# cczls1991/DL_Biomass

Hardware: NVIDIA B200
Metric: train tree-clouds/sec @10k pts (higher is better)
Workload: dtype bf16

## Files before the change

### dl_biomass_b200/csrc/sa_tc.cu

```cuda
#include <cuda.h>
#include <math.h>

#include "tc_common.cuh"

namespace b2pn {
namespace tc {

constexpr int R = 128;
constexpr int KC = 64;
constexpr int NUM_EPI = 256;
constexpr int NUM_LOAD = 128;
constexpr int LOAD_GROUPS = 2;
constexpr int MMA_WARP = (NUM_EPI + LOAD_GROUPS * NUM_LOAD) / 32;
constexpr int NT = NUM_EPI + LOAD_GROUPS * NUM_LOAD + 32;
constexpr int NT_TMA = 2 * NUM_EPI + 64;
constexpr int PROD_WARP_TMA = MMA_WARP + 1;
constexpr int NT_WIDE = 2 * NUM_EPI + 32 + NUM_LOAD;
constexpr int B_BYTES = R * LINE_BYTES;

constexpr unsigned GI_NONE = 0x00ffffffu;
__device__ __forceinline__ int gi_seg(unsigned b) { return (int)(b & 0xffffffu); }
__device__ __forceinline__ bool gi_none(unsigned b) { return (b & 0xffffffu) == 0xffffffu; }
__device__ __forceinline__ int gi_slot0(unsigned b) { return (int)((b >> 24) & 7u) << 3; }
__device__ __forceinline__ int gi_nv(unsigned b) { return (int)((b >> 27) & 15u); }
// ... 244 lines not shown
    }
    static __device__ __forceinline__ uint64_t b_desc(uint32_t b_saddr, int ks) { return smem_desc_sw128(b_saddr + ks * 32, 16, ATOM_BYTES); }
};

constexpr int GATHER_ROWS = 64;
__global__ void __launch_bounds__(256) gather_l1_tc_kernel(GatherLoaderTC gl, const int64_t *rows_dev, int kg, int64_t ld,
                                                          __nv_bfloat16 *G)
{
    extern __shared__ __align__(16) unsigned char gth_smem[];
    __nv_bfloat16 *S = reinterpret_cast<__nv_bfloat16 *>(gth_smem);
    const int64_t rows = rows_dev ? *rows_dev : gl.rm.rows;
    gl.resolve(rows);
    const int64_t r0 = (int64_t)blockIdx.x * GATHER_ROWS;
    if (r0 >= (rows + 127) / 128 * 128) return;
    const int kg8 = (kg + 7) & ~7;
    const int rl = threadIdx.x & 63, q = threadIdx.x >> 6;
    gl.set_row(r0 + rl);
    for (int kk = q * 8; kk < kg8; kk += 32) {
        const uint4 v = gl.chunk(kk);
        const __nv_bfloat16 *e = reinterpret_cast<const __nv_bfloat16 *>(&v);
#pragma unroll
        for (int j = 0; j < 8; ++j) S[(kk + j) * GATHER_ROWS + rl] = e[j];
    }
    __syncthreads();
    for (int i = threadIdx.x; i < kg8 * 8; i += 256) {
        const int k = i >> 3, part = i & 7;
        if (k < kg)
            *reinterpret_cast<uint4 *>(G + (int64_t)k * ld + r0 + part * 8) =
                *reinterpret_cast<const uint4 *>(S + k * GATHER_ROWS + part * 8);
    }
}

template <int MODE>
struct FeatSource {
    static constexpr bool USES_TMA = false;
    static constexpr bool SCATTER = false;
    RowMapTC rm;
    const __nv_bfloat16 *t;
    int C;
    int64_t ld;
    int act;
    int ones_line;
    const float *gamma;
    const float *beta;
    int out_fmt;
    __device__ __forceinline__ uint4 pack_out(const float (&f)[8]) const { return out_fmt == FMT_F16 ? pack8h(f) : pack8(f); }
    __device__ __forceinline__ void resolve(int64_t r) { rm.resolve(r); }
    __device__ __forceinline__ uint4 chunk_i(int ch, int64_t r8, unsigned inf) const
    {
        const int nv = gi_nv(inf);
        float f[8];
        if (ch == ones_line) {
#pragma unroll
            for (int e = 0; e < 8; ++e) f[e] = e < nv ? 1.f : 0.f;
            return pack_out(f);
        }
        const bool live = ch < C && nv > 0;
        uint4 raw = make_uint4(0u, 0u, 0u, 0u);
        if (!live) return raw;
        raw = __ldg(reinterpret_cast<const uint4 *>(t + (int64_t)ch * ld + r8));
        if (MODE == 0 && nv == 8 && out_fmt == FMT_F16) return raw;
        unpack8h(raw, f);
        float ga = 1.f, be = 0.f;
        if (MODE != 0) {
            ga = gamma[ch];
            be = beta[ch];
        }
#pragma unroll
        for (int e = 0; e < 8; ++e) {
            float v = f[e];
            if (MODE != 0) {
                v = fmaf(v, ga, be);
                if (act == B2PN_ACT_RELU) v = fmaxf(v, 0.f);
            }
            f[e] = e < nv ? v : 0.f;
        }
        return pack_out(f);
    }
};

struct TmaSource {
    static constexpr bool USES_TMA = true;
    static constexpr bool SCATTER = false;
    RowMapTC rm;
    __device__ __forceinline__ void resolve(int64_t r) { rm.resolve(r); }
    __device__ __forceinline__ uint4 chunk_i(int, int64_t, unsigned) const { return make_uint4(0u, 0u, 0u, 0u); }
};

struct RouteSource {
    static constexpr bool USES_TMA = false;
    RowMapTC rm;
    const float *dout;
    const int32_t *arg;
    int C;
    __device__ __forceinline__ void resolve(int64_t r) { rm.resolve(r); }
    static constexpr bool SCATTER = true;
    int vec;
    struct Quad {
        int4 a;
        float4 d;
    };
    __device__ __forceinline__ bool starts(unsigned inf, int ch4) const { return ch4 < C && gi_nv(inf) > 0 && gi_slot0(inf) == 0; }
    __device__ __forceinline__ void load_quad(unsigned inf, int ch4, Quad &q) const
    {
        const bool first = starts(inf, ch4);
        const int64_t idx = first ? (int64_t)gi_seg(inf) * C + ch4 : 0;
        if (vec) {
            q.a = __ldg(reinterpret_cast<const int4 *>(arg + idx));
            q.d = __ldg(reinterpret_cast<const float4 *>(dout + idx));
        } else {
            const int64_t last = (first ? (int64_t)gi_seg(inf) * C : 0) + C - 1;
            q.a = make_int4(__ldg(arg + idx), __ldg(arg + min(idx + 1, last)), __ldg(arg + min(idx + 2, last)), __ldg(arg + min(idx + 3, last)));
            q.d = make_float4(__ldg(dout + idx), __ldg(dout + min(idx + 1, last)), __ldg(dout + min(idx + 2, last)),
                              __ldg(dout + min(idx + 3, last)));
        }
    }
    __device__ __forceinline__ void store_quad(const Quad &q, bool first, int ch4, int g, uint32_t blk, int l0) const
    {
        const int a[4] = {q.a.x, q.a.y, q.a.z, q.a.w};
        const float d[4] = {q.d.x, q.d.y, q.d.z, q.d.w};
#pragma unroll
        for (int e = 0; e < 4; ++e) {
            const unsigned row = (unsigned)(g * 8 + a[e]);
            const unsigned ok = (first && ch4 + e < C && a[e] >= 0 && row < 64u) ? 1u : 0u;
            const uint32_t line = (uint32_t)(l0 + e);
            const uint32_t addr = blk + line * LINE_BYTES + ((((row >> 3) & 7u) ^ (line & 7u)) << 4) + ((row & 7u) << 1);
            const unsigned short gb = __bfloat16_as_ushort(__float2bfloat16(d[e]));
            asm volatile("{\n\t.reg .pred p;\n\tsetp.ne.u32 p, %2, 0;\n\t@p st.shared.b16 [%0], %1;\n\t}" ::"r"(addr), "h"(gb), "r"(ok)
                         : "memory");
        }
    }
    template <int NTHR = NUM_LOAD>
    static __device__ __forceinline__ void zero_tile(uint32_t base, int bytes, int lt)
    {
        for (int o = lt * 16; o < bytes; o += NTHR * 16)
            asm volatile("st.shared.v4.b32 [%0], {%1, %1, %1, %1};" ::"r"(base + (uint32_t)o), "r"(0u) : "memory");
    }
    template <int NTHR = NUM_LOAD>
    static __device__ __forceinline__ void group_barrier(int id) { asm volatile("bar.sync %0, %1;" ::"r"(id), "n"(NTHR) : "memory"); }
    __device__ __forceinline__ uint4 chunk_i(int ch, int64_t, unsigned inf) const
    {
        const bool live = ch < C && gi_nv(inf) > 0;
        const int64_t idx = live ? (int64_t)gi_seg(inf) * C + ch : 0;
        const int a = __ldg(arg + idx) - gi_slot0(inf);
        const float d = __ldg(dout + idx);
        const bool hit = live && a >= 0 && a < 8;
        const unsigned short gb = __bfloat16_as_ushort(__float2bfloat16(d));
        const unsigned w = (a & 1) ? ((unsigned)gb << 16) : (unsigned)gb;
        const int q = hit ? (a >> 1) : -1;
        uint4 v;
        v.x = q == 0 ? w : 0u;
        v.y = q == 1 ? w : 0u;
        v.z = q == 2 ? w : 0u;
        v.w = q == 3 ? w : 0u;
        return v;
    }
};

template <class SRC, bool WIDE_ = false>
struct FeatLoaderTC {
    static constexpr bool B_MN = true;
    static constexpr bool USES_TMA = false;
    static constexpr bool WIDE = WIDE_;
    static constexpr bool PIPELINED = SRC::SCATTER;
    SRC src;
    int64_t row0;
    unsigned inf[8];
    static constexpr int PIPE_GROUPS = 2;
    unsigned qinf[2], qraw1[2], qraw2[2], qdead1, qdead2;
    struct Item {
        typename SRC::Quad q[2];
        unsigned first;
    };
// ... 802 lines not shown
    static constexpr bool USES_TMA = true;
    int c;
    int ones_box;
    const float *fix_gamma;
    const float *fix_beta;
    int fix_act;
    __device__ __forceinline__ uint4 convert(const uint4 &raw, int c16, int ng) const
    {
        const int ch = ng * 256 + (c16 >> 3);
        if (fix_gamma == nullptr || ch >= c) return f16_to_bf16_chunk(raw);
        const float ga = __ldg(fix_gamma + ch), be = __ldg(fix_beta + ch);
        float f[8];
        unpack8h(raw, f);
#pragma unroll
        for (int e = 0; e < 8; ++e) {
            f[e] = fmaf(f[e], ga, be);
            if (fix_act == B2PN_ACT_RELU) f[e] = fmaxf(f[e], 0.f);
        }
        return pack8(f);
    }
    static __host__ __device__ int bytes(int nb_lines) { return ((nb_lines + 63) / 64) * 64 * LINE_BYTES; }
    __device__ __forceinline__ void resolve(int64_t) {}
    __device__ __forceinline__ void fill(uint8_t *, int, int64_t, int, int, const unsigned (&)[8]) {}
    __device__ __forceinline__ int landed_lines(int ng) const
    {
        const int ch0 = ng * 256;
        const int left = c - ch0;
        const int boxes = left <= 0 ? 0 : ((left < 256 ? left : 256) + 63) >> 6;
        const bool ones_here = ones_box && c >= ch0 && c < ch0 + 256;
        const int tensor_lines = boxes * 64;
        return ones_here ? max(tensor_lines, c - ch0 + 16) : tensor_lines;
    }
    __device__ __forceinline__ unsigned fill_tma(uint8_t *B, int64_t r0, int ng, const TmaMap *map_x, const TmaMap *map_v,
                                                 uint64_t *bar) const
    {
        const int ch0 = ng * 256;
        const int left = c - ch0;
        const int boxes = left <= 0 ? 0 : ((left < 256 ? left : 256) + 63) >> 6;
        const bool ones_here = ones_box && c >= ch0 && c < ch0 + 256;
        const unsigned bytes = (unsigned)((boxes * 64 + (ones_here ? 16 : 0)) * LINE_BYTES);
        mbar_expect_tx(bar, bytes);
        for (int blk = 0; blk < boxes; ++blk) tma_load_2d(B + blk * (64 * LINE_BYTES), map_x, (int)r0, ch0 + blk * 64, bar);
        if (ones_here) tma_load_2d(B + (c - ch0) * LINE_BYTES, map_v, (int)r0, 0, bar);
        return bytes;
    }
    static __device__ __forceinline__ uint64_t b_desc(uint32_t b_saddr, int ks) { return smem_desc_sw128(b_saddr + ks * 32, 16, ATOM_BYTES); }
};

struct LineFillGather {
    static constexpr bool B_MN = true;
    static constexpr bool USES_TMA = false;
    GatherLoaderTC g;
    static __host__ __device__ int bytes(int nb_lines) { return ((nb_lines + 63) / 64) * 64 * LINE_BYTES; }
    __device__ __forceinline__ void resolve(int64_t r) { g.resolve(r); }
    __device__ __forceinline__ void fill(uint8_t *B, int lt, int64_t r0, int ng, int nb_lines, const unsigned (&inf)[8])
    {
        const int rl = lt >> 1, half = lt & 1;
        g.set_row(r0 + rl);
        const int nblk = (nb_lines + 63) / 64;
        for (int blk = 0; blk < nblk; ++blk) {
#pragma unroll
            for (int c = 0; c < 4; ++c) {
                const int cc = half * 4 + c;
                *reinterpret_cast<uint4 *>(B + blk * (64 * LINE_BYTES) + line_chunk_off(rl, cc)) =
                    g.chunk(ng * 256 + blk * 64 + cc * 8);
            }
        }
    }
    static __device__ __forceinline__ uint64_t b_desc(uint32_t b_saddr, int ks)
    {
        return smem_desc_sw128(b_saddr + ks * (16 * LINE_BYTES), 64 * LINE_BYTES, ATOM_BYTES);
    }
};

template <int MTA>
struct DwPlan {
    static constexpr int A_BYTES = MTA * 128 * LINE_BYTES;
    static constexpr int MAX_STAGES = 8;
    static constexpr int SMEM_BUDGET = 222 * 1024;
};

template <int MTA, class YS, class XF>
__global__ void __launch_bounds__(NT, 1) tc_dw_kernel(const DwParams p, YS ys, XF xf, const __grid_constant__ TmaMap tmap_y,
                                                       const __grid_constant__ TmaMap tmap_x, const __grid_constant__ TmaMap tmap_v)
{
    using P = DwPlan<MTA>;
    const int nst = p.stages, sbytes = p.stage_bytes;
    extern __shared__ uint8_t smem_raw[];
    uint8_t *smem = reinterpret_cast<uint8_t *>((reinterpret_cast<uintptr_t>(smem_raw) + 1023) & ~(uintptr_t)1023);
    uint64_t *full = reinterpret_cast<uint64_t *>(smem + nst * sbytes);
    uint64_t *empty = full + nst;
    uint64_t *done = empty + nst;
    uint64_t *xland = done + 1;
    uint32_t *tmem_holder = reinterpret_cast<uint32_t *>(xland + nst);

    const int tid = threadIdx.x, warp = tid >> 5, lane = tid & 31;
    const int split = blockIdx.x, mg = blockIdx.y, ng = blockIdx.z;
    constexpr int TCOLS = MTA * 256;
    const int64_t rows = p.rows_dev ? *p.rows_dev : p.rows;
    ys.resolve(rows);
    xf.resolve(rows);
    const int64_t chunks = (rows + 63) / 64;
    const int64_t cps = (chunks + gridDim.x - 1) / gridDim.x;
    const int64_t c_beg = (int64_t)split * cps;
    const int64_t c_end = min(chunks, c_beg + cps);
    const int64_t nchunks = c_end > c_beg ? c_end - c_beg : 0;
    const int nb_lines = min(256, p.nbl_total - ng * 256);

    if (tid == 0) {
        for (int s = 0; s < nst; ++s) {
            mbar_init(&full[s], YS::SCATTER ? 2 * NUM_LOAD : NUM_LOAD);
            mbar_init(&empty[s], 1);
            mbar_init(&xland[s], 1);
        }
        mbar_init(done, 1);
        fence_barrier_init();
    }
    if (warp == MMA_WARP) tmem_alloc<TCOLS>(tmem_holder);
    tc_fence_before();
    __syncthreads();
    tc_fence_after();
    const uint32_t tmem_base = *tmem_holder;

    constexpr bool ANY_TMA = YS::USES_TMA || XF::USES_TMA;
    constexpr bool DEDICATED = ANY_TMA && !YS::SCATTER;
    auto issue = [&](int64_t i) {
        const int s = (int)(i % nst);
        const uint32_t ph = (uint32_t)(i / nst) & 1u;
        uint8_t *A = smem + s * sbytes;
        uint8_t *B = A + P::A_BYTES;
        const int64_t r0 = (c_beg + i) * 64;
        mbar_wait(&empty[s], ph ^ 1u);
        if constexpr (YS::USES_TMA) {
            mbar_expect_tx(&full[s], P::A_BYTES);
#pragma unroll
            for (int m = 0; m < MTA * 2; ++m)
                tma_load_2d(A + m * (64 * LINE_BYTES), &tmap_y, (int)r0, mg * (MTA * 128) + m * 64, &full[s]);
        }
        if constexpr (XF::USES_TMA) {
            xf.fill_tma(B, r0, ng, &tmap_x, &tmap_v, &xland[s]);
            mbar_arrive(&xland[s]);
        }
    };
    constexpr int NG = DEDICATED ? LOAD_GROUPS + 1 : LOAD_GROUPS;
    if ((warp >= NUM_EPI / 32 && warp < MMA_WARP) || (DEDICATED && warp < 4)) {
        const int grp = warp < 4 ? LOAD_GROUPS : (tid - NUM_EPI) / NUM_LOAD;
        const int lt = warp < 4 ? tid : (tid - NUM_EPI) % NUM_LOAD;
        auto load_inf = [&](unsigned (&inf)[8], int64_t r0) {
            if (ys.rm.seg_mode) {
#pragma unroll
                for (int g = 0; g < 8; ++g) inf[g] = ys.rm.info(r0 + g * 8);
            } else {
#pragma unroll
                for (int g = 0; g < 8; ++g) inf[g] = ys.rm.info_slots(r0 + g * 8);
            }
        };
        unsigned inf[8], infn[8];
        if (grp < nchunks) load_inf(inf, (c_beg + grp) * 64);
        const int ahead = nst / NG > 1 ? nst / NG : 1;
        int64_t iss = grp;
        for (int64_t i = grp; i < nchunks; i += NG) {
            const int s = (int)(i % nst);
            const uint32_t ph = (uint32_t)(i / nst) & 1u;
            uint8_t *A = smem + s * sbytes;
            uint8_t *B = A + P::A_BYTES;
            const int64_t r0 = (c_beg + i) * 64;
            if (i + NG < nchunks) load_inf(infn, (c_beg + i + NG) * 64);
            if constexpr (ANY_TMA && !DEDICATED) {
                if (lt == 0)
                    for (; iss < nchunks && iss < i + (int64_t)ahead * NG; iss += NG) issue(iss);
            }
            if constexpr (!YS::USES_TMA) {
                if constexpr (YS::SCATTER) {
                } else {
                    uint4 v[MTA][8];
#pragma unroll
                    for (int m = 0; m < MTA; ++m) {
                        const int ch = mg * (MTA * 128) + m * 128 + lt;
#pragma unroll
                        for (int g = 0; g < 8; ++g) v[m][g] = ys.chunk_i(ch, r0 + g * 8, inf[g]);
                    }
                    mbar_wait(&empty[s], ph ^ 1u);
#pragma unroll
                    for (int m = 0; m < MTA; ++m) {
                        const int line = m * 128 + lt;
#pragma unroll
                        for (int g = 0; g < 8; ++g) *reinterpret_cast<uint4 *>(A + line_chunk_off(line, g)) = v[m][g];
                    }
                }
            }
            if constexpr (XF::USES_TMA) {
                mbar_wait(&empty[s], ph ^ 1u);
                mbar_wait(&xland[s], ph);
                const int nchunk16 = xf.landed_lines(ng) * 8;
                for (int c = lt; c < nchunk16; c += NUM_LOAD) {
                    uint4 *q = reinterpret_cast<uint4 *>(B) + c;
                    *q = xf.convert(*q, c, ng);
                }
            } else {
                if constexpr (YS::USES_TMA || YS::SCATTER) mbar_wait(&empty[s], ph ^ 1u);
                xf.fill(B, lt, r0, ng, nb_lines, inf);
            }
            fence_proxy_async_smem();
            mbar_arrive(&full[s]);
#pragma unroll
            for (int g = 0; g < 8; ++g) inf[g] = infn[g];
        }
    } else if (warp == MMA_WARP) {
        if (lane == 0 && nchunks > 0) {
            const uint32_t idesc = idesc_bf16(128, nb_lines, false, XF::B_MN);
            for (int64_t i = 0; i < nchunks; ++i) {
                const int s = (int)(i % nst);
                const uint32_t ph = (uint32_t)(i / nst) & 1u;
                mbar_wait(&full[s], ph);
                tc_fence_after();
                const uint32_t a_s = smem_u32(smem + s * sbytes);
                const uint32_t b_s = a_s + P::A_BYTES;
#pragma unroll
                for (int mt = 0; mt < MTA; ++mt) {
#pragma unroll
                    for (int ks = 0; ks < 4; ++ks) {
                        const uint64_t ad = smem_desc_sw128(a_s + mt * (128 * LINE_BYTES) + ks * 32, 16, ATOM_BYTES);
                        const uint64_t bd = XF::b_desc(b_s, ks);
                        umma_bf16(tmem_base + mt * 256, ad, bd, idesc, (i | ks) != 0);
                    }
                }
                umma_commit(&empty[s]);
            }
            umma_commit(done);
        }
    } else {
        if constexpr (DEDICATED) {
            if (warp == 4 && lane == 0)
                for (int64_t i = 0; i < nchunks; ++i) issue(i);
        }
        if constexpr (YS::SCATTER) {
            const int grp = tid / NUM_LOAD;
            const int lt = tid % NUM_LOAD;
            constexpr int NQ = MTA * 32, NI = MTA * 2;
            RouteSource::Quad qd[NI];
            unsigned qi[NI], r1[NI], r2[NI], r3[NI], d1 = 0u, d2 = 0u, d3 = 0u;
            auto q_fetch = [&](unsigned (&w)[NI], unsigned &dead, int64_t i) {
                dead = 0u;
#pragma unroll
                for (int k = 0; k < NI; ++k) {
                    if (i < nchunks) {
                        const int64_t r8 = (c_beg + i) * 64 + ((lt + NUM_LOAD * k) / NQ) * 8;
                        w[k] = __ldg(ys.rm.rgrp + (r8 >> 3));
                        dead |= (r8 >= ys.rm.rows ? 1u : 0u) << k;
                    } else {
                        w[k] = GI_NONE;
                        dead |= 1u << k;
                    }
                }
            };
            auto q_norm = [&](const unsigned (&w)[NI], unsigned dead) {
#pragma unroll
                for (int k = 0; k < NI; ++k) qi[k] = (((dead >> k) & 1u) || gi_none(w[k])) ? GI_NONE : w[k];
            };
            auto q_load = [&]() {
#pragma unroll
                for (int k = 0; k < NI; ++k) ys.load_quad(qi[k], mg * (MTA * 128) + ((lt + NUM_LOAD * k) % NQ) * 4, qd[k]);
            };
            auto q_prefetch = [&](const unsigned (&w)[NI], unsigned dead) {
#pragma unroll
                for (int k = 0; k < NI; ++k) {
                    const int q = (lt + NUM_LOAD * k) % NQ;
                    const int ch4 = mg * (MTA * 128) + q * 4;
                    if ((q & 7) != 0 || ((dead >> k) & 1u) || gi_none(w[k]) || gi_nv(w[k]) == 0 || gi_slot0(w[k]) != 0 || ch4 >= ys.C) continue;
                    const int64_t idx = (int64_t)gi_seg(w[k]) * ys.C + ch4;
                    asm volatile("prefetch.global.L2 [%0];" ::"l"(ys.arg + idx));
                    asm volatile("prefetch.global.L2 [%0];" ::"l"(ys.dout + idx));
                }
            };
#pragma unroll
            for (int k = 0; k < NI; ++k) qi[k] = r1[k] = r2[k] = r3[k] = GI_NONE;
            if (grp < nchunks) {
                q_fetch(r1, d1, grp);
                q_norm(r1, d1);
                q_load();
                q_fetch(r1, d1, grp + LOAD_GROUPS);
                q_fetch(r2, d2, grp + 2 * LOAD_GROUPS);
            }
            for (int64_t i = grp; i < nchunks; i += LOAD_GROUPS) {
                const int s = (int)(i % nst);
                const uint32_t ph = (uint32_t)(i / nst) & 1u;
                uint8_t *A = smem + s * sbytes;
                q_fetch(r3, d3, i + 3 * LOAD_GROUPS);
                q_prefetch(r2, d2);
                mbar_wait(&empty[s], ph ^ 1u);
                RouteSource::zero_tile(smem_u32(A), P::A_BYTES, lt);
                RouteSource::group_barrier(1 + grp);
#pragma unroll
                for (int k = 0; k < NI; ++k) {
                    const int l0 = ((lt + NUM_LOAD * k) % NQ) * 4, g = (lt + NUM_LOAD * k) / NQ;
                    const int ch4 = mg * (MTA * 128) + l0;
                    ys.store_quad(qd[k], ys.starts(qi[k], ch4), ch4, g, smem_u32(A), l0);
                }
                fence_proxy_async_smem();
                mbar_arrive(&full[s]);
                if (i + LOAD_GROUPS < nchunks) {
                    q_norm(r1, d1);
                    q_load();
                }
#pragma unroll
                for (int k = 0; k < NI; ++k) {
                    r1[k] = r2[k];
                    r2[k] = r3[k];
                }
                d1 = d2, d2 = d3;
            }
        }
// ... 263 lines not shown

__global__ void bn_bwd_finalize_tc_kernel(const double *partial, int gx, int C, int cpad, const CountArg count, int training,
                                          float *grad_gamma, float *grad_beta, float *sbar)
{
    const int c = (blockIdx.x * blockDim.x + threadIdx.x) >> 5;
    if (c >= C) return;
    double S, Q;
    warp_sum_partials(partial, gx, cpad, c, S, Q);
    if ((threadIdx.x & 31) == 0) {
        const double E = count.get();
        if (grad_beta) grad_beta[c] = (float)S;
        if (grad_gamma) grad_gamma[c] = (float)Q;
        sbar[c] = (training && E > 0) ? (float)(S / E) : 0.f;
        sbar[C + c] = (training && E > 0) ? (float)(Q / E) : 0.f;
    }
}

template <bool CLOUDS>
__global__ void route_grad_tc_kernel(RowMapTC rm, const int64_t *rows_dev, const float *dout, const int32_t *arg, int C, int64_t ld,
                                     __nv_bfloat16 *dh)
{
    if (rows_dev) rm.rows = *rows_dev;
    const int64_t groups = (rm.rows + 127) / 128 * 16;
    const int64_t total = groups * C;
    for (int64_t i = (int64_t)blockIdx.x * blockDim.x + threadIdx.x; i < total; i += (int64_t)gridDim.x * blockDim.x) {
        const int ch = (int)(i / groups);
        const int64_t g = i - (int64_t)ch * groups;
        const unsigned inf = rm.info(g * 8);
        uint4 v = make_uint4(0u, 0u, 0u, 0u);
        if (CLOUDS) {
            float f[8];
            bool any = false;
#pragma unroll
            for (int e = 0; e < 8; ++e) {
                const int64_t row = g * 8 + e;
                f[e] = 0.f;
                if (e < gi_nv(inf)) {
                    const int64_t sg = __ldg(rm.batch + row);
                    if ((int64_t)__ldg(arg + sg * C + ch) == row) {
                        f[e] = __ldg(dout + sg * C + ch);
                        any = true;
                    }
                }
            }
            if (any) v = pack8(f);
        } else if (gi_nv(inf) > 0) {
            const int64_t m = gi_seg(inf);
            const int a = __ldg(arg + m * C + ch) - gi_slot0(inf);
            if (a >= 0 && a < 8) {
                const unsigned short gb = __bfloat16_as_ushort(__float2bfloat16(__ldg(dout + m * C + ch)));
                const unsigned w = (a & 1) ? ((unsigned)gb << 16) : (unsigned)gb;
                const int q = a >> 1;
                v.x = q == 0 ? w : 0u;
                v.y = q == 1 ? w : 0u;
                v.z = q == 2 ? w : 0u;
                v.w = q == 3 ? w : 0u;
            }
        }
        *reinterpret_cast<uint4 *>(dh + (int64_t)ch * ld + g * 8) = v;
    }
}

__global__ void bn_bwd_apply_tc_kernel(RowMapTC rm, const int64_t *rows_dev, __nv_bfloat16 *dz, const __nv_bfloat16 *z, int C,
                                       int64_t ld, const float *scale, const float *sbar)
{
    if (rows_dev) rm.rows = *rows_dev;
    const int64_t groups = (rm.rows + 127) / 128 * 16;
    const int64_t total = groups * C;
    for (int64_t i = (int64_t)blockIdx.x * blockDim.x + threadIdx.x; i < total; i += (int64_t)gridDim.x * blockDim.x) {
        const int ch = (int)(i / groups);
        const int64_t r8 = (i - (int64_t)ch * groups) * 8;
        const int nv = rm.valid8(r8);
        uint4 *p = reinterpret_cast<uint4 *>(dz + (int64_t)ch * ld + r8);
        if (nv == 0) {
            *p = make_uint4(0u, 0u, 0u, 0u);
            continue;
        }
        float d[8], zf[8];
        unpack8(*p, d);
        unpack8h(__ldg(reinterpret_cast<const uint4 *>(z + (int64_t)ch * ld + r8)), zf);
        const float sc = scale[ch];
        const float s1 = sbar[ch], s2 = sbar[C + ch];
#pragma unroll
        for (int e = 0; e < 8; ++e) d[e] = e < nv ? sc * (d[e] - s1 - zf[e] * s2) : 0.f;
        *p = pack8(d);
    }
}

struct DwReduceJob {
    const float *partial;
    int splits, n_out, k_total, use_map;
    InCols cols;
    int k_true, ones_idx;
    float *grad_w, *grad_b;
};
struct DwReduceJobs {
    DwReduceJob j[3];
};
__global__ void dw_reduce_flat_tc_kernel(const DwReduceJobs jobs)
{
    const DwReduceJob &jb = jobs.j[blockIdx.y];
    const int k_true = jb.k_true, k_total = jb.k_total, n_out = jb.n_out, splits = jb.splits;
    const int64_t i = (int64_t)blockIdx.x * blockDim.x + threadIdx.x;
    if (i >= (int64_t)n_out * (k_true + 1)) return;
    const int n = (int)(i / (k_true + 1));
    const int k = (int)(i - (int64_t)n * (k_true + 1));
    int c0 = -1, c1 = -1;
    if (k == k_true) {
        c0 = jb.ones_idx;
    } else if (!jb.use_map) {
        c0 = k;
    } else {
        const int nx = jb.cols.nx();
        if (k < jb.cols.c_in) {
            c0 = k;
            c1 = jb.cols.x_f32 ? k + jb.cols.c_in : -1;
        } else {
            c0 = nx + (k - jb.cols.c_in);
            c1 = c0 + 3;
        }
    }
    const int64_t stride = (int64_t)n_out * k_total;
    const float *base = jb.partial + (int64_t)n * k_total;
    constexpr int U = 16;
    double acc[U];
#pragma unroll
    for (int u = 0; u < U; ++u) acc[u] = 0.0;
    int p = 0;
    for (; p + U <= splits; p += U) {
#pragma unroll
        for (int u = 0; u < U; ++u) {
            const float *row = base + (int64_t)(p + u) * stride;
            float v = row[c0];
            if (c1 >= 0) v += row[c1];
            acc[u] += (double)v;
        }
    }
    for (; p < splits; ++p) {
        const float *row = base + (int64_t)p * stride;
        acc[0] += (double)row[c0];
        if (c1 >= 0) acc[0] += (double)row[c1];
    }
#pragma unroll
    for (int w = U / 2; w > 0; w >>= 1)
#pragma unroll
        for (int u = 0; u < w; ++u) acc[u] += acc[u + w];
    const double sum = acc[0];
    if (k == k_true) {
        if (jb.grad_b) jb.grad_b[n] = (float)sum;
    } else if (jb.grad_w) {
        jb.grad_w[(int64_t)n * k_true + k] = (float)sum;
    }
}

constexpr int DWR_WARPS = 8;
constexpr int DWR_MAX_SPLITS = 160;
__global__ void __launch_bounds__(32 * DWR_WARPS) dw_reduce_tc_kernel(const DwReduceJobs jobs)
{
    const DwReduceJob &jb = jobs.j[blockIdx.y];
    const int k_true = jb.k_true, k_total = jb.k_total, n_out = jb.n_out, splits = jb.splits;
    const int w = threadIdx.y;
    const int64_t i = (int64_t)blockIdx.x * 32 + threadIdx.x;
    const bool live = i < (int64_t)n_out * (k_true + 1);
    const int n = live ? (int)(i / (k_true + 1)) : 0;
    const int k = live ? (int)(i - (int64_t)n * (k_true + 1)) : 0;
    int c0 = 0, c1 = -1;
    if (k == k_true) {
// ... 421 lines not shown
        p2.rows = ra.cap; p2.rows_dev = ra.dev; p2.ld = s.ld;
        p2.bias_a = a.mlp.b[0]; p2.mean_a = bn1; p2.rstd_a = bn1 + s.cmax; p2.gamma_a = a.mlp.gamma[0]; p2.beta_a = a.mlp.beta[0];
        p2.act = a.mlp.act; p2.z_out = (__half *)z1; p2.a_out = (__half *)a.a1;
        p2.partial = f.partial; p2.cpad = s.cpad; p2.rgrp = a.rgrp;
        const int nks1 = (s.k1 - (p2.kc_in - 1) * KC) >= KC ? 4 : (s.k1 - (p2.kc_in - 1) * KC + 15) / 16;
        if (p2.kc_in == 1 && nks1 == 1 && p2.kc_mid == 1) rc = launch(tc_chain_train_kernel<2, 1, 1, 1, 1>, p2, map_g1);
        else if (p2.kc_in == 3 && nks1 == 1 && p2.kc_mid == 2) rc = launch(tc_chain_train_kernel<2, 3, 1, 2, 1>, p2, map_g1);
        else rc = launch(tc_chain_train_kernel<2, -1, -1, -1, -1>, p2, map_g1);
        if (rc) return rc;
        bn_fwd_finalize_tc_kernel<<<(s.c2 + 3) / 4, 128, 0, st>>>(f.partial, 4 * gx, s.c2, s.cpad, count, train, a.mlp.b[1], a.mlp.gamma[1],
                                                                     a.mlp.beta[1], a.mlp.running_mean[1], a.mlp.running_var[1],
                                                                     a.mlp.num_batches_tracked[1], a.mlp.eps, a.mlp.momentum, bn2, s.cmax);
        note_launch();
        TmaMap map_in3;
        if ((rc = make_tma_feature_major(&map_in3, a.a1 ? a.a1 : (const void *)z1, s.c1, s.ld))) return rc;
        ChainTrainParams p3 = {};
        p3.w_img[0] = f.pk[1].img; p3.w_bytes[0] = (int)f.pk[1].bytes;
        p3.w_img[1] = f.pk[2].img; p3.w_bytes[1] = (int)f.pk[2].bytes;
        p3.k_in = s.c1; p3.kc_in = f.pk[1].num_kc; p3.kc_mid = f.pk[2].num_kc;
        p3.c_a = s.c2; p3.c_b = s.c3; p3.mt_b = f.pk[2].MT; p3.dup_a = s.c2 == 64;
        p3.rows = ra.cap; p3.rows_dev = ra.dev; p3.ld = s.ld;
        p3.bias_a = a.mlp.b[1]; p3.mean_a = bn2; p3.rstd_a = bn2 + s.cmax; p3.gamma_a = a.mlp.gamma[1]; p3.beta_a = a.mlp.beta[1];
        p3.act = a.mlp.act; p3.z_out = (__half *)z2; p3.a_out = (__half *)a.a2;
        if (!a.a1) {
            p3.fix_gamma = a.mlp.gamma[0];
            p3.fix_beta = a.mlp.beta[0];
        }
        p3.bias_b = a.mlp.b[2]; p3.out = a.out; p3.arg = a.arg; p3.out16 = (__half *)a.out_bf16; p3.rgrp = a.rgrp;
        if (p3.kc_in == 1 && p3.kc_mid == 1 && p3.mt_b == 1) rc = launch(tc_chain_train_kernel<3, 1, 4, 1, 1>, p3, map_in3);
        else if (p3.kc_in == 2 && p3.kc_mid == 2 && p3.mt_b == 2) rc = launch(tc_chain_train_kernel<3, 2, 4, 2, 2>, p3, map_in3);
        else rc = launch(tc_chain_train_kernel<3, -1, -1, -1, -1>, p3, map_in3);
        if (rc) return rc;
        B2PN_LAUNCH_CHECK();
        return B2PN_OK;
    }
    if (s.rows > 0) {
        NormStoreEpTC e = {s.c1, a.mlp.b[0], bn1, bn1 + s.cmax, a.mlp.gamma[0], a.mlp.beta[0], a.mlp.act, rm};
        TmaMap mz, ma;
        if ((rc = make_tma_feature_major(&mz, z1, s.c1, s.ld, 32))) return rc;
        if ((rc = make_tma_feature_major(&ma, a.a1, s.c1, s.ld, 32))) return rc;
        rc = use_g1 ? launch_by_mt(f.pk[0], ra, tl1, e, e, st, map_g1, mz, ma) : launch_by_mt(f.pk[0], ra, gl, e, e, st, kNoMap, mz, ma);
        if (rc) return rc;
    }
    TmaFeatLoader l2, l3;
    TmaMap map_a1, map_a2;
    if ((rc = make_tma_feature_major(&map_a1, a.a1, s.c1, s.ld))) return rc;
    if ((rc = make_tma_feature_major(&map_a2, a.a2, s.c2, s.ld))) return rc;
    if (train && s.rows > 0) {
        StatsEpTC<1> e1 = {s.c2, f.partial, s.cpad, 4};
        StatsEpTC<2> e2 = {s.c2, f.partial, s.cpad, 4};
        if ((rc = launch_by_mt(f.pk[1], ra, l2, e1, e2, st, map_a1))) return rc;
    }
    bn_fwd_finalize_tc_kernel<<<(s.c2 + 3) / 4, 128, 0, st>>>(f.partial, 4 * grid_x_for(f.pk[1], s.tiles), s.c2, s.cpad, count, train,
                                                                 a.mlp.b[1], a.mlp.gamma[1], a.mlp.beta[1], a.mlp.running_mean[1],
                                                                 a.mlp.running_var[1], a.mlp.num_batches_tracked[1], a.mlp.eps,
                                                                 a.mlp.momentum, bn2, s.cmax);
    note_launch();
    if (s.rows > 0) {
        NormStoreEpTC e = {s.c2, a.mlp.b[1], bn2, bn2 + s.cmax, a.mlp.gamma[1], a.mlp.beta[1], a.mlp.act, rm};
        TmaMap mz, ma;
        if ((rc = make_tma_feature_major(&mz, z2, s.c2, s.ld, 32))) return rc;
        if ((rc = make_tma_feature_major(&ma, a.a2, s.c2, s.ld, 32))) return rc;
        if ((rc = launch_by_mt(f.pk[1], ra, l2, e, e, st, map_a1, mz, ma))) return rc;
    }
    if (a.seg_mode == B2PN_SEG_SLOTS) {
        SlotMaxEpTC e = {a.out, a.arg, s.c3, a.mlp.b[2], a.rgrp, s.rows, (__half *)a.out_bf16};
        if ((rc = launch_by_mt(f.pk[2], ra, l3, e, e, st, map_a2))) return rc;
    } else {
        const int64_t n = a.n_dst * (int64_t)s.c3;
        B2PN_CUDA(cudaMemsetAsync(f.keys, 0, n * sizeof(unsigned long long), st));
        if (s.rows > 0) {
            CloudMaxEpTC e = {f.keys, s.c3, a.mlp.b[2], a.batch, s.rows};
            if ((rc = launch_by_mt(f.pk[2], ra, l3, e, e, st, map_a2))) return rc;
        }
        unpack_keys_tc_kernel<<<(unsigned)((n + 255) / 256), 256, 0, st>>>(f.keys, a.out, a.arg, n);
        note_launch();
    }
    B2PN_LAUNCH_CHECK();
    return B2PN_OK;
}

template <class YS, class XF>
static int launch_dw(const YS &ys, const XF &xf, int n_out, int k_total, const ShapesTC &s, const RowsArg &ra, float *dwp,
                     cudaStream_t st, const TmaMap &map_y = kNoMap, const TmaMap &map_x = kNoMap, const TmaMap &map_v = kNoMap)
{
    const DwPlanHost d = plan_dw(n_out, k_total, s.ld);
    DwParams p = {ra.cap, ra.dev, n_out, d.nbl_total, d.k_stride, dwp, dw_atomic() ? 1 : 0, 0, 0};
    if (dw_atomic()) {
        cudaError_t em = cudaMemsetAsync(dwp, 0, (size_t)n_out * d.k_stride * sizeof(float), st);
        if (em != cudaSuccess) return (int)em;
    }
    const int nb_max = d.nbl_total < 256 ? d.nbl_total : 256;
    const int b_bytes = (int)align_up(XF::bytes(nb_max), 1024);
    dim3 grid((unsigned)d.splits, (unsigned)d.num_mg, (unsigned)d.num_ng);
    cudaError_t e;
    auto plan = [&](int a_bytes) {
        p.stage_bytes = a_bytes + b_bytes;
        p.stages = (DwPlan<1>::SMEM_BUDGET - 1280) / p.stage_bytes;
        if (p.stages > DwPlan<1>::MAX_STAGES) p.stages = DwPlan<1>::MAX_STAGES;
        if (p.stages < 2) p.stages = 2;
        return p.stages * p.stage_bytes + 256 + 1024;
    };
    if (d.MTA == 1) {
        auto kern = tc_dw_kernel<1, YS, XF>;
        const int smem = plan(DwPlan<1>::A_BYTES);
        static SmemAttrSlot slot = {};
        e = ensure_dynamic_smem(kern, smem, slot);
        if (e != cudaSuccess) return (int)e;
        kern<<<grid, NT, smem, st>>>(p, ys, xf, map_y, map_x, map_v);
    } else {
        auto kern = tc_dw_kernel<2, YS, XF>;
        const int smem = plan(DwPlan<2>::A_BYTES);
        static SmemAttrSlot slot = {};
        e = ensure_dynamic_smem(kern, smem, slot);
        if (e != cudaSuccess) return (int)e;
        kern<<<grid, NT, smem, st>>>(p, ys, xf, map_y, map_x, map_v);
    }
    note_launch();
    e = cudaPeekAtLastError();
    return e == cudaSuccess ? 0 : (int)e;
}

static unsigned apply_grid(int64_t ld, int C)
{
    const int64_t n = (ld / 8) * C;
    int64_t blocks = (n + 255) / 256;
    const int64_t cap = (int64_t)sm_count() * 8;
    if (blocks > cap) blocks = cap;
    return (unsigned)(blocks > 0 ? blocks : 1);
}

static DwReduceJob dw_reduce_job(const float *dwp, int n_out, int k_total, const InCols *map, int k_true, int ones_idx,
                                 const ShapesTC &s, float *gw, float *gb)
{
    const DwPlanHost d = plan_dw(n_out, k_total, s.ld);
    DwReduceJob j = {dwp, dw_atomic() ? 1 : d.splits, n_out, d.k_stride, map ? 1 : 0, map ? *map : InCols{0, 0}, k_true, ones_idx, gw, gb};
    return j;
}
static void launch_dw_reduces(const DwReduceJob *jobs, int n, cudaStream_t st)
{
    DwReduceJobs dj;
    int64_t mx = 0;
    for (int i = 0; i < 3; ++i) {
        dj.j[i] = jobs[i < n ? i : 0];
        const int64_t tot = (int64_t)dj.j[i].n_out * (dj.j[i].k_true + 1);
        mx = tot > mx ? tot : mx;
    }
    if (mx <= 16384)
        dw_reduce_tc_kernel<<<dim3((unsigned)((mx + 31) / 32), (unsigned)n), dim3(32, DWR_WARPS), 0, st>>>(dj);
    else
        dw_reduce_flat_tc_kernel<<<dim3((unsigned)((mx + 127) / 128), (unsigned)n), 128, 0, st>>>(dj);
    note_launch();
}

int sa_backward_bf16(const b2pn_sa_args &a, const b2pn_sa_grads &g, cudaStream_t st)
{
    int rc = check_args_tc(a);
    if (rc) return rc;
    if (!g.grad_out) return B2PN_EINVAL;
    const ShapesTC s = shapes_tc(a);
    if (a.n_dst == 0 || s.rows == 0) return B2PN_OK;
    if (a.workspace_bytes < sa_workspace_bytes_bf16(a, 1) || !a.workspace) return B2PN_EINVAL;
    WsTC ws(a.workspace);
    BwdWsTC b = carve_bwd_tc(a, s, ws);
    const RowMapTC rm = rowmap_tc(a, s);
    const RowsArg ra = rowsarg_tc(a, s);
    const __nv_bfloat16 *z1 = (const __nv_bfloat16 *)a.h1, *z2 = (const __nv_bfloat16 *)a.h2;
    float *bn1 = a.bn, *bn2 = a.bn + 4 * s.cmax;
    const bool need_dx = g.grad_x != nullptr && a.c_in > 0;

    {
        const PackJob jobs[3] = {pack_job(a.mlp.w[2], s.c2, s.c3, 1, s.c2, nullptr, b.pkT[2]),
                                 pack_job(a.mlp.w[1], s.c1, s.c2, 1, s.c1, nullptr, b.pkT[1]),
                                 pack_job(a.mlp.w[0], a.c_in, s.c1, 1, s.c0, nullptr, b.pkT[0])};
        launch_packs(jobs, need_dx ? 3 : 2, st);
    }
    const CountArg count = {a.seg_mode == B2PN_SEG_SLOTS ? a.num_rows + 1 : nullptr, (double)s.rows};

    MaskSumsStoreEpTC<1> e31 = {s.c2, a.mlp.gamma[1], a.mlp.beta[1], a.mlp.act, b.partial, s.cpad, 4};
    MaskSumsStoreEpTC<2> e32 = {s.c2, a.mlp.gamma[1], a.mlp.beta[1], a.mlp.act, b.partial, s.cpad, 4};
    TmaMap mdz2, mz2;
    if ((rc = make_tma_feature_major(&mdz2, b.dz2, s.c2, s.ld, 32))) return rc;
    if ((rc = make_tma_feature_major(&mz2, z2, s.c2, s.ld, 32))) return rc;
    LineFillK<FeatSource<1>> xa2 = {{rm, z2, s.c2, s.ld, a.mlp.act, s.c2, a.mlp.gamma[1], a.mlp.beta[1], FMT_BF16}};
    TmaMap map_v = kNoMap, map_a1 = kNoMap, map_a2 = kNoMap;
    const bool tma_x = a.row_valid != nullptr;
    const bool tma_x2 = tma_x && s.c2 % 64 == 0 && (s.c2 % 256) + 16 <= 256, tma_x1 = tma_x && s.c1 % 64 == 0 && (s.c1 % 256) + 16 <= 256;
    if (tma_x2 || tma_x1) {
        if ((rc = make_tma_row_valid(&map_v, a.row_valid, s.ld))) return rc;
    }
    const bool x_from_z = a.a1 == nullptr;
    if (x_from_z && !(tma_x1 && tma_x2 && a.seg_mode == B2PN_SEG_SLOTS)) return B2PN_EINVAL;
    if (tma_x2 && (rc = make_tma_feature_major(&map_a2, x_from_z ? (const void *)z2 : a.a2, s.c2, s.ld))) return rc;
    if (tma_x1 && (rc = make_tma_feature_major(&map_a1, x_from_z ? (const void *)z1 : a.a1, s.c1, s.ld))) return rc;
    if (a.seg_mode == B2PN_SEG_CLOUDS) {
        route_grad_tc_kernel<true><<<apply_grid(s.ld, s.c3), 256, 0, st>>>(rm, ra.dev, g.grad_out, a.arg, s.c3, s.ld, b.dh3);
        note_launch();
        TmaMap map3;
        if ((rc = make_tma_feature_major(&map3, b.dh3, s.c3, s.ld))) return rc;
        TmaFeatLoader bl;
        if ((rc = launch_by_mt(b.pkT[2], ra, bl, e31, e32, st, map3, mdz2, mz2))) return rc;
        TmaSource y3 = {rm};
        if (tma_x2) {
            TmaFill xt = {s.c2, 1, nullptr, nullptr, 0};
            rc = launch_dw(y3, xt, s.c3, s.c2 + 1, s, ra, b.dwp[2], st, map3, map_a2, map_v);
        } else {
            rc = launch_dw(y3, xa2, s.c3, s.c2 + 1, s, ra, b.dwp[2], st, map3);
        }
        if (rc) return rc;
    } else {
        const int vec = (s.c3 % 4 == 0 && ((uintptr_t)g.grad_out | (uintptr_t)a.arg) % 16 == 0) ? 1 : 0;
        RouteSource rs = {rm, g.grad_out, a.arg, s.c3, vec};
        FeatLoaderTC<RouteSource, true> bl = {rs};
        if ((rc = launch_by_mt(b.pkT[2], ra, bl, e31, e32, st, kNoMap, mdz2, mz2))) return rc;
        if (tma_x2) {
            TmaFill xt = {s.c2, 1, x_from_z ? a.mlp.gamma[1] : nullptr, a.mlp.beta[1], a.mlp.act};
            rc = launch_dw(rs, xt, s.c3, s.c2 + 1, s, ra, b.dwp[2], st, kNoMap, map_a2, map_v);
        } else {
            rc = launch_dw(rs, xa2, s.c3, s.c2 + 1, s, ra, b.dwp[2], st);
        }
        if (rc) return rc;
    }
    bn_bwd_finalize_tc_kernel<<<(s.c2 + 3) / 4, 128, 0, st>>>(b.partial, 4 * grid_x_for(b.pkT[2], s.tiles), s.c2, s.cpad, count,
                                                                 a.training, g.grad_gamma[1], g.grad_beta[1], b.sbar);
    note_launch();
    {
        bn_bwd_apply_tc_kernel<<<apply_grid(s.ld, s.c2), 256, 0, st>>>(rm, ra.dev, b.dz2, z2, s.c2, s.ld, bn2 + 2 * s.cmax, b.sbar);
        note_launch();
    }
    TmaMap map2, map1;
    if ((rc = make_tma_feature_major(&map2, b.dz2, s.c2, s.ld))) return rc;
    if ((rc = make_tma_feature_major(&map1, b.dz1, s.c1, s.ld))) return rc;
    TmaSource y2 = {rm};
    {
        TmaFeatLoader bl;
        MaskSumsStoreEpTC<1> e1 = {s.c1, a.mlp.gamma[0], a.mlp.beta[0], a.mlp.act, b.partial, s.cpad, 4};
        MaskSumsStoreEpTC<2> e2 = {s.c1, a.mlp.gamma[0], a.mlp.beta[0], a.mlp.act, b.partial, s.cpad, 4};
        TmaMap mdz1, mz1;
        if ((rc = make_tma_feature_major(&mdz1, b.dz1, s.c1, s.ld, 32))) return rc;
        if ((rc = make_tma_feature_major(&mz1, z1, s.c1, s.ld, 32))) return rc;
        if ((rc = launch_by_mt(b.pkT[1], ra, bl, e1, e2, st, map2, mdz1, mz1))) return rc;
        if (tma_x1) {
            TmaFill xt = {s.c1, 1, x_from_z ? a.mlp.gamma[0] : nullptr, a.mlp.beta[0], a.mlp.act};
            rc = launch_dw(y2, xt, s.c2, s.c1 + 1, s, ra, b.dwp[1], st, map2, map_a1, map_v);
        } else {
            LineFillK<FeatSource<1>> xa1 = {{rm, z1, s.c1, s.ld, a.mlp.act, s.c1, a.mlp.gamma[0], a.mlp.beta[0], FMT_BF16}};
            rc = launch_dw(y2, xa1, s.c2, s.c1 + 1, s, ra, b.dwp[1], st, map2);
        }
        if (rc) return rc;
    }
    bn_bwd_finalize_tc_kernel<<<(s.c1 + 3) / 4, 128, 0, st>>>(b.partial, 4 * grid_x_for(b.pkT[1], s.tiles), s.c1, s.cpad, count,
                                                                 a.training, g.grad_gamma[0], g.grad_beta[0], b.sbar);
    note_launch();
    {
        bn_bwd_apply_tc_kernel<<<apply_grid(s.ld, s.c1), 256, 0, st>>>(rm, ra.dev, b.dz1, z1, s.c1, s.ld, bn1 + 2 * s.cmax, b.sbar);
        note_launch();
    }
    TmaSource y1 = {rm};
    {
        if (l1_materialised(a, s)) {
            TmaMap map_g1;
            if ((rc = make_tma_feature_major(&map_g1, a.g1, s.k1 + 1, s.ld))) return rc;
            TmaFill xt = {s.k1 + 1, 0, nullptr, nullptr, 0};
            rc = launch_dw(y1, xt, s.c1, s.k1 + 1, s, ra, b.dwp[0], st, map1, map_g1, kNoMap);
        } else {
            LineFillGather xg = {{rm, a.x, s.cols, a.pos_src, a.pos_dst, s.k1, FMT_BF16}};
            rc = launch_dw(y1, xg, s.c1, s.k1 + 1, s, ra, b.dwp[0], st, map1);
        }
        if (rc) return rc;
        const DwReduceJob jobs[3] = {dw_reduce_job(b.dwp[2], s.c3, s.c2 + 1, nullptr, s.c2, s.c2, s, g.grad_w[2], g.grad_b[2]),
                                     dw_reduce_job(b.dwp[1], s.c2, s.c1 + 1, nullptr, s.c1, s.c1, s, g.grad_w[1], g.grad_b[1]),
                                     dw_reduce_job(b.dwp[0], s.c1, s.k1 + 1, &s.cols, s.c0, s.k1, s, g.grad_w[0], g.grad_b[0])};
        launch_dw_reduces(jobs, 3, st);
    }
    if (need_dx) {
        TmaFeatLoader bl;
        const int64_t nx = a.n_src * (int64_t)a.c_in;
        if (b.dxi) B2PN_CUDA(cudaMemsetAsync(b.dxi, 0, (size_t)nx * sizeof(long long), st));
        else if (a.seg_mode == B2PN_SEG_SLOTS) B2PN_CUDA(cudaMemsetAsync(g.grad_x, 0, (size_t)nx * sizeof(float), st));
        ScatterEpTC e = {rm, g.grad_x, a.c_in, b.dxi};
        if ((rc = launch_by_mt(b.pkT[0], ra, bl, e, e, st, map1))) return rc;
        if (b.dxi) {
            fixed_to_f32_kernel<<<(unsigned)((nx + 255) / 256), 256, 0, st>>>(b.dxi, g.grad_x, nx);
            note_launch();
        }
    }
    B2PN_LAUNCH_CHECK();
    return B2PN_OK;
}

}
}
```

Measured before the change: 5954.

## Fuse batchnorm-backward dz formation into weight-gradient kernel for slot mode

In slot segment mode, the separate bn_bwd_apply kernels are skipped. The dW tensor-core kernel instead TMA-loads both the upstream gradient and z tiles, forms dz in shared memory in the loader warps, and TMA-stores dz back for later consumers. The layer-2 dW launch is moved ahead of the dX GEMM so it produces dz2 before that GEMM reads it. For layer 1 the store happens only when dx is needed. This removes two elementwise kernel launches and one full read-modify-write pass per layer. In exchange the kernel uses extra shared memory for the z tile when it does not fit alongside y, does more work in the loader stage, and adds a store/wait in the MMA warp.

```diff
diff --git a/dl_biomass_b200/csrc/sa_tc.cu b/dl_biomass_b200/csrc/sa_tc.cu
--- a/dl_biomass_b200/csrc/sa_tc.cu
+++ b/dl_biomass_b200/csrc/sa_tc.cu
@@ -350,13 +350,55 @@
 struct TmaSource {
     static constexpr bool USES_TMA = true;
     static constexpr bool SCATTER = false;
+    static constexpr bool FORMS_DZ = false;
     RowMapTC rm;
     __device__ __forceinline__ void resolve(int64_t r) { rm.resolve(r); }
     __device__ __forceinline__ uint4 chunk_i(int, int64_t, unsigned) const { return make_uint4(0u, 0u, 0u, 0u); }
 };
 
+__device__ __forceinline__ float bn_bwd_dz(float g, float zhat, float scale, float s1, float s2)
+{
+    return scale * fmaf(zhat, -s2, g - s1);
+}
+
+struct DzSource {
+    static constexpr bool USES_TMA = true;
+    static constexpr bool SCATTER = false;
+    static constexpr bool FORMS_DZ = true;
+    RowMapTC rm;
+    int C;
+    const float *scale;
+    const float *sbar;
+    int store;
+    __device__ __forceinline__ void resolve(int64_t r) { rm.resolve(r); }
+    __device__ __forceinline__ uint4 chunk_i(int, int64_t, unsigned) const { return make_uint4(0u, 0u, 0u, 0u); }
+    __device__ __forceinline__ int boxes(int ch0, int lines) const { return min(lines, max(C - ch0, 0) + 63) >> 6; }
+    __host__ __device__ bool z_in_tile(int mta, int num_mg) const { return num_mg == 1 && C <= mta * 64; }
+    __device__ __forceinline__ void form(uint8_t *Y, const uint8_t *Z, int lt, int nthreads, int ch0, int lines, unsigned nvw) const
+    {
+        const int n16 = min(lines, C - ch0) * 8;
+        for (int c = lt; c < n16; c += nthreads) {
+            const int line = c >> 3, g = (c & 7) ^ (line & 7), nv = (int)(nvw >> (4 * g)) & 15;
+            uint4 *p = reinterpret_cast<uint4 *>(Y) + c;
+            if (nv == 0) {
+                *p = make_uint4(0u, 0u, 0u, 0u);
+                continue;
+            }
+            const int ch = ch0 + line;
+            float d[8], zf[8];
+            unpack8(*p, d);
+            unpack8h(reinterpret_cast<const uint4 *>(Z)[c], zf);
+            const float sc = __ldg(scale + ch), s1 = __ldg(sbar + ch), s2 = __ldg(sbar + C + ch);
+#pragma unroll
+            for (int e = 0; e < 8; ++e) d[e] = e < nv ? bn_bwd_dz(d[e], zf[e], sc, s1, s2) : 0.f;
+            *p = pack8(d);
+        }
+    }
+};
+
 struct RouteSource {
     static constexpr bool USES_TMA = false;
+    static constexpr bool FORMS_DZ = false;
     RowMapTC rm;
     const float *dout;
     const int32_t *arg;
@@ -1325,7 +1367,8 @@
 
 template <int MTA, class YS, class XF>
 __global__ void __launch_bounds__(NT, 1) tc_dw_kernel(const DwParams p, YS ys, XF xf, const __grid_constant__ TmaMap tmap_y,
-                                                       const __grid_constant__ TmaMap tmap_x, const __grid_constant__ TmaMap tmap_v)
+                                                       const __grid_constant__ TmaMap tmap_x, const __grid_constant__ TmaMap tmap_v,
+                                                       const __grid_constant__ TmaMap tmap_z)
 {
     using P = DwPlan<MTA>;
     const int nst = p.stages, sbytes = p.stage_bytes;
@@ -1359,6 +1402,19 @@
         mbar_init(done, 1);
         fence_barrier_init();
     }
+    const int ych0 = mg * (MTA * 128);
+    int y_bytes = P::A_BYTES, zoff = 0, nbox = 0;
+    if constexpr (YS::FORMS_DZ) {
+        nbox = ys.boxes(ych0, MTA * 128);
+        const bool zin = ys.z_in_tile(MTA, gridDim.y);
+        zoff = zin ? nbox * (64 * LINE_BYTES) : P::A_BYTES;
+        y_bytes = zin ? P::A_BYTES : 2 * P::A_BYTES;
+        const int from = (zin ? 2 : 1) * nbox * 64;
+        for (int s = 0; s < nst; ++s)
+            for (int c = from * 8 + tid; c < MTA * 128 * 8; c += NT)
+                reinterpret_cast<uint4 *>(smem + s * sbytes)[c] = make_uint4(0u, 0u, 0u, 0u);
+        fence_proxy_async_smem();
+    }
     if (warp == MMA_WARP) tmem_alloc<TCOLS>(tmem_holder);
     tc_fence_before();
     __syncthreads();
@@ -1371,19 +1427,23 @@
         const int s = (int)(i % nst);
         const uint32_t ph = (uint32_t)(i / nst) & 1u;
         uint8_t *A = smem + s * sbytes;
-        uint8_t *B = A + P::A_BYTES;
+        uint8_t *B = A + y_bytes;
         const int64_t r0 = (c_beg + i) * 64;
         mbar_wait(&empty[s], ph ^ 1u);
-        if constexpr (YS::USES_TMA) {
+        if constexpr (YS::FORMS_DZ) {
+            mbar_expect_tx(&xland[s], (unsigned)(nbox * 2 * 64 * LINE_BYTES));
+            for (int m = 0; m < nbox; ++m) {
+                tma_load_2d(A + m * (64 * LINE_BYTES), &tmap_y, (int)r0, ych0 + m * 64, &xland[s]);
+                tma_load_2d(A + zoff + m * (64 * LINE_BYTES), &tmap_z, (int)r0, ych0 + m * 64, &xland[s]);
+            }
+        } else if constexpr (YS::USES_TMA) {
             mbar_expect_tx(&full[s], P::A_BYTES);
 #pragma unroll
             for (int m = 0; m < MTA * 2; ++m)
-                tma_load_2d(A + m * (64 * LINE_BYTES), &tmap_y, (int)r0, mg * (MTA * 128) + m * 64, &full[s]);
-        }
-        if constexpr (XF::USES_TMA) {
-            xf.fill_tma(B, r0, ng, &tmap_x, &tmap_v, &xland[s]);
-            mbar_arrive(&xland[s]);
-        }
+                tma_load_2d(A + m * (64 * LINE_BYTES), &tmap_y, (int)r0, ych0 + m * 64, &full[s]);
+        }
+        if constexpr (XF::USES_TMA) xf.fill_tma(B, r0, ng, &tmap_x, &tmap_v, &xland[s]);
+        if constexpr (XF::USES_TMA || YS::FORMS_DZ) mbar_arrive(&xland[s]);
     };
     constexpr int NG = DEDICATED ? LOAD_GROUPS + 1 : LOAD_GROUPS;
     if ((warp >= NUM_EPI / 32 && warp < MMA_WARP) || (DEDICATED && warp < 4)) {
@@ -1406,7 +1466,7 @@
             const int s = (int)(i % nst);
             const uint32_t ph = (uint32_t)(i / nst) & 1u;
             uint8_t *A = smem + s * sbytes;
-            uint8_t *B = A + P::A_BYTES;
+            uint8_t *B = A + y_bytes;
             const int64_t r0 = (c_beg + i) * 64;
             if (i + NG < nchunks) load_inf(infn, (c_beg + i + NG) * 64);
             if constexpr (ANY_TMA && !DEDICATED) {
@@ -1432,17 +1492,21 @@
                     }
                 }
             }
+            if constexpr (XF::USES_TMA || YS::USES_TMA || YS::SCATTER) mbar_wait(&empty[s], ph ^ 1u);
+            if constexpr (!XF::USES_TMA) xf.fill(B, lt, r0, ng, nb_lines, inf);
+            if constexpr (XF::USES_TMA || YS::FORMS_DZ) mbar_wait(&xland[s], ph);
+            if constexpr (YS::FORMS_DZ) {
+                unsigned nvw = 0u;
+#pragma unroll
+                for (int g = 0; g < 8; ++g) nvw |= (unsigned)gi_nv(inf[g]) << (4 * g);
+                ys.form(A, A + zoff, lt, NUM_LOAD, ych0, MTA * 128, nvw);
+            }
             if constexpr (XF::USES_TMA) {
-                mbar_wait(&empty[s], ph ^ 1u);
-                mbar_wait(&xland[s], ph);
                 const int nchunk16 = xf.landed_lines(ng) * 8;
                 for (int c = lt; c < nchunk16; c += NUM_LOAD) {
                     uint4 *q = reinterpret_cast<uint4 *>(B) + c;
                     *q = xf.convert(*q, c, ng);
                 }
-            } else {
-                if constexpr (YS::USES_TMA || YS::SCATTER) mbar_wait(&empty[s], ph ^ 1u);
-                xf.fill(B, lt, r0, ng, nb_lines, inf);
             }
             fence_proxy_async_smem();
             mbar_arrive(&full[s]);
@@ -1458,7 +1522,16 @@
                 mbar_wait(&full[s], ph);
                 tc_fence_after();
                 const uint32_t a_s = smem_u32(smem + s * sbytes);
-                const uint32_t b_s = a_s + P::A_BYTES;
+                const uint32_t b_s = a_s + y_bytes;
+                bool stored = false;
+                if constexpr (YS::FORMS_DZ) {
+                    if (ys.store) {
+                        for (int m = 0; m < nbox; ++m)
+                            tma_store_2d(&tmap_y, smem + s * sbytes + m * (64 * LINE_BYTES), (int)((c_beg + i) * 64), ych0 + m * 64);
+                        bulk_commit_group();
+                        stored = true;
+                    }
+                }
 #pragma unroll
                 for (int mt = 0; mt < MTA; ++mt) {
 #pragma unroll
@@ -1468,9 +1541,11 @@
                         umma_bf16(tmem_base + mt * 256, ad, bd, idesc, (i | ks) != 0);
                     }
                 }
+                if (stored) bulk_wait_read_all();
                 umma_commit(&empty[s]);
             }
             umma_commit(done);
+            if constexpr (YS::FORMS_DZ) bulk_wait_all();
         }
     } else {
         if constexpr (DEDICATED) {
@@ -1900,7 +1975,7 @@
         const float sc = scale[ch];
         const float s1 = sbar[ch], s2 = sbar[C + ch];
 #pragma unroll
-        for (int e = 0; e < 8; ++e) d[e] = e < nv ? sc * (d[e] - s1 - zf[e] * s2) : 0.f;
+        for (int e = 0; e < 8; ++e) d[e] = e < nv ? bn_bwd_dz(d[e], zf[e], sc, s1, s2) : 0.f;
         *p = pack8(d);
     }
 }
@@ -2488,7 +2563,8 @@
 
 template <class YS, class XF>
 static int launch_dw(const YS &ys, const XF &xf, int n_out, int k_total, const ShapesTC &s, const RowsArg &ra, float *dwp,
-                     cudaStream_t st, const TmaMap &map_y = kNoMap, const TmaMap &map_x = kNoMap, const TmaMap &map_v = kNoMap)
+                     cudaStream_t st, const TmaMap &map_y = kNoMap, const TmaMap &map_x = kNoMap, const TmaMap &map_v = kNoMap,
+                     const TmaMap &map_z = kNoMap)
 {
     const DwPlanHost d = plan_dw(n_out, k_total, s.ld);
     DwParams p = {ra.cap, ra.dev, n_out, d.nbl_total, d.k_stride, dwp, dw_atomic() ? 1 : 0, 0, 0};
@@ -2507,20 +2583,22 @@
         if (p.stages < 2) p.stages = 2;
         return p.stages * p.stage_bytes + 256 + 1024;
     };
+    int y_tiles = 1;
+    if constexpr (YS::FORMS_DZ) y_tiles = ys.z_in_tile(d.MTA, d.num_mg) ? 1 : 2;
     if (d.MTA == 1) {
         auto kern = tc_dw_kernel<1, YS, XF>;
-        const int smem = plan(DwPlan<1>::A_BYTES);
+        const int smem = plan(y_tiles * DwPlan<1>::A_BYTES);
         static SmemAttrSlot slot = {};
         e = ensure_dynamic_smem(kern, smem, slot);
         if (e != cudaSuccess) return (int)e;
-        kern<<<grid, NT, smem, st>>>(p, ys, xf, map_y, map_x, map_v);
+        kern<<<grid, NT, smem, st>>>(p, ys, xf, map_y, map_x, map_v, map_z);
     } else {
         auto kern = tc_dw_kernel<2, YS, XF>;
-        const int smem = plan(DwPlan<2>::A_BYTES);
+        const int smem = plan(y_tiles * DwPlan<2>::A_BYTES);
         static SmemAttrSlot slot = {};
         e = ensure_dynamic_smem(kern, smem, slot);
         if (e != cudaSuccess) return (int)e;
-        kern<<<grid, NT, smem, st>>>(p, ys, xf, map_y, map_x, map_v);
+        kern<<<grid, NT, smem, st>>>(p, ys, xf, map_y, map_x, map_v, map_z);
     }
     note_launch();
     e = cudaPeekAtLastError();
@@ -2630,15 +2708,33 @@
     bn_bwd_finalize_tc_kernel<<<(s.c2 + 3) / 4, 128, 0, st>>>(b.partial, 4 * grid_x_for(b.pkT[2], s.tiles), s.c2, s.cpad, count,
                                                                  a.training, g.grad_gamma[1], g.grad_beta[1], b.sbar);
     note_launch();
-    {
+    const bool dz_in_dw = a.seg_mode == B2PN_SEG_SLOTS;
+    if (!dz_in_dw) {
         bn_bwd_apply_tc_kernel<<<apply_grid(s.ld, s.c2), 256, 0, st>>>(rm, ra.dev, b.dz2, z2, s.c2, s.ld, bn2 + 2 * s.cmax, b.sbar);
         note_launch();
     }
     TmaMap map2, map1;
     if ((rc = make_tma_feature_major(&map2, b.dz2, s.c2, s.ld))) return rc;
     if ((rc = make_tma_feature_major(&map1, b.dz1, s.c1, s.ld))) return rc;
-    TmaSource y2 = {rm};
-    {
+    {
+        TmaMap map_z2 = kNoMap;
+        if (dz_in_dw && (rc = make_tma_feature_major(&map_z2, z2, s.c2, s.ld))) return rc;
+        auto dw2 = [&](const auto &y2) {
+            if (tma_x1) {
+                TmaFill xt = {s.c1, 1, x_from_z ? a.mlp.gamma[0] : nullptr, a.mlp.beta[0], a.mlp.act};
+                return launch_dw(y2, xt, s.c2, s.c1 + 1, s, ra, b.dwp[1], st, map2, map_a1, map_v, map_z2);
+            }
+            LineFillK<FeatSource<1>> xa1 = {{rm, z1, s.c1, s.ld, a.mlp.act, s.c1, a.mlp.gamma[0], a.mlp.beta[0], FMT_BF16}};
+            return launch_dw(y2, xa1, s.c2, s.c1 + 1, s, ra, b.dwp[1], st, map2, kNoMap, kNoMap, map_z2);
+        };
+        if (dz_in_dw) {
+            const DzSource y2 = {rm, s.c2, bn2 + 2 * s.cmax, b.sbar, 1};
+            rc = dw2(y2);
+        } else {
+            const TmaSource y2 = {rm};
+            rc = dw2(y2);
+        }
+        if (rc) return rc;
         TmaFeatLoader bl;
         MaskSumsStoreEpTC<1> e1 = {s.c1, a.mlp.gamma[0], a.mlp.beta[0], a.mlp.act, b.partial, s.cpad, 4};
         MaskSumsStoreEpTC<2> e2 = {s.c1, a.mlp.gamma[0], a.mlp.beta[0], a.mlp.act, b.partial, s.cpad, 4};
@@ -2646,32 +2742,34 @@
         if ((rc = make_tma_feature_major(&mdz1, b.dz1, s.c1, s.ld, 32))) return rc;
         if ((rc = make_tma_feature_major(&mz1, z1, s.c1, s.ld, 32))) return rc;
         if ((rc = launch_by_mt(b.pkT[1], ra, bl, e1, e2, st, map2, mdz1, mz1))) return rc;
-        if (tma_x1) {
-            TmaFill xt = {s.c1, 1, x_from_z ? a.mlp.gamma[0] : nullptr, a.mlp.beta[0], a.mlp.act};
-            rc = launch_dw(y2, xt, s.c2, s.c1 + 1, s, ra, b.dwp[1], st, map2, map_a1, map_v);
-        } else {
-            LineFillK<FeatSource<1>> xa1 = {{rm, z1, s.c1, s.ld, a.mlp.act, s.c1, a.mlp.gamma[0], a.mlp.beta[0], FMT_BF16}};
-            rc = launch_dw(y2, xa1, s.c2, s.c1 + 1, s, ra, b.dwp[1], st, map2);
-        }
-        if (rc) return rc;
     }
     bn_bwd_finalize_tc_kernel<<<(s.c1 + 3) / 4, 128, 0, st>>>(b.partial, 4 * grid_x_for(b.pkT[1], s.tiles), s.c1, s.cpad, count,
                                                                  a.training, g.grad_gamma[0], g.grad_beta[0], b.sbar);
     note_launch();
-    {
+    if (!dz_in_dw) {
         bn_bwd_apply_tc_kernel<<<apply_grid(s.ld, s.c1), 256, 0, st>>>(rm, ra.dev, b.dz1, z1, s.c1, s.ld, bn1 + 2 * s.cmax, b.sbar);
         note_launch();
     }
-    TmaSource y1 = {rm};
-    {
-        if (l1_materialised(a, s)) {
-            TmaMap map_g1;
-            if ((rc = make_tma_feature_major(&map_g1, a.g1, s.k1 + 1, s.ld))) return rc;
-            TmaFill xt = {s.k1 + 1, 0, nullptr, nullptr, 0};
-            rc = launch_dw(y1, xt, s.c1, s.k1 + 1, s, ra, b.dwp[0], st, map1, map_g1, kNoMap);
+    {
+        TmaMap map_z1 = kNoMap;
+        if (dz_in_dw && (rc = make_tma_feature_major(&map_z1, z1, s.c1, s.ld))) return rc;
+        auto dw1 = [&](const auto &y1) {
+            if (l1_materialised(a, s)) {
+                TmaMap map_g1;
+                int e = make_tma_feature_major(&map_g1, a.g1, s.k1 + 1, s.ld);
+                if (e) return e;
+                TmaFill xt = {s.k1 + 1, 0, nullptr, nullptr, 0};
+                return launch_dw(y1, xt, s.c1, s.k1 + 1, s, ra, b.dwp[0], st, map1, map_g1, kNoMap, map_z1);
+            }
+            LineFillGather xg = {{rm, a.x, s.cols, a.pos_src, a.pos_dst, s.k1, FMT_BF16}};
+            return launch_dw(y1, xg, s.c1, s.k1 + 1, s, ra, b.dwp[0], st, map1, kNoMap, kNoMap, map_z1);
+        };
+        if (dz_in_dw) {
+            const DzSource y1 = {rm, s.c1, bn1 + 2 * s.cmax, b.sbar, need_dx ? 1 : 0};
+            rc = dw1(y1);
         } else {
-            LineFillGather xg = {{rm, a.x, s.cols, a.pos_src, a.pos_dst, s.k1, FMT_BF16}};
-            rc = launch_dw(y1, xg, s.c1, s.k1 + 1, s, ra, b.dwp[0], st, map1);
+            const TmaSource y1 = {rm};
+            rc = dw1(y1);
         }
         if (rc) return rc;
         const DwReduceJob jobs[3] = {dw_reduce_job(b.dwp[2], s.c3, s.c2 + 1, nullptr, s.c2, s.c2, s, g.grad_w[2], g.grad_b[2]),
```

After: 6129 (median of 6 runs). 1.03x the previous value.
